# NVlabs/CenterPose

Hardware: AMD Instinct MI355X
Metric: images/sec at 512x512 DLA-34 (backbone + heat-map decode + post-process + PnP) (higher is better)
Workload: dtype f32 via split-f16 (f16x3) MFMA, f32 accumulate

## Files before the change

centerpose_amd/csrc/dcn16t.hip:

```cpp
#include <type_traits>

#include "dcn_patch_common.h"
#include "patch16_common.h"
#include "upadd_common.h"

namespace {

constexpr int T_TH = PATCH_TH, T_TW = PATCH_TW, T_HALO = 3;
constexpr int T_PW = T_TW + 2 * T_HALO, T_PH = T_TH + 2 * T_HALO, T_NPIX = T_PH * T_PW;
constexpr int T_CK = 16;
constexpr int T_PSTR = T_CK * 4 + 16;
constexpr int T_ECAP = 184;
constexpr int T_NPIX_ALL = T_NPIX + T_ECAP + T_PW + 1;
constexpr int T_NSTEP = 9;
constexpr int T_RQ = T_PW * (T_CK / 4);
constexpr int T_ROUNDS = T_PH / 2;
static_assert(2 * T_RQ <= 256 && T_PH % 2 == 0, "two patch rows per staging round");
static_assert(T_NPIX_ALL * T_PSTR + T_ECAP * 24 + 64 <= 53 * 1024, "three workgroups per CU");
static_assert((T_PSTR / 16) % 2 == 1, "odd pixel pitch in bank groups");

struct TGeo {
    static constexpr int PH = T_PH, PW = T_PW, HALO = T_HALO, ECAP = T_ECAP;
    static __device__ __forceinline__ int corner(int qy, int qx) { return qy * T_PW + qx; }
    static __device__ __forceinline__ int spare(int e) { return T_NPIX + e; }
};

template <int NT, bool UPADD = false>
__global__ __launch_bounds__(256, 3) void dcn16t_kernel(const ConvParams p, const int tiles_m, const int tiles_n) {
    typedef Frag<32> F;
    typedef F::acc_t acc_t;
    static_assert(NT == 2, "64-wide N tile");
    __shared__ __attribute__((aligned(16))) unsigned char patch[T_NPIX_ALL * T_PSTR];
    __shared__ int exc_key[T_ECAP];
    __shared__ int exc_goff[T_ECAP];
    __shared__ __attribute__((aligned(16))) float exc_w[T_ECAP][4];
    __shared__ int exc_count;

    const int tid = threadIdx.x, lane = tid & 63;
    const int wid = __builtin_amdgcn_readfirstlane(tid >> 6);
    const int lrow = lane >> 5, lcol = lane & 31;
    const int tile = tile_of_block(tiles_m, tiles_n);
    const int tn = tile % tiles_n;
    int tm = tile / tiles_n;
    const int txs = p.W / T_TW, tys = p.H / T_TH;
    const int tx0 = (tm % txs) * T_TW;
    tm /= txs;
    const int ty0 = (tm % tys) * T_TH, b = tm / tys;
    const AmaxRaw amax_raw = conv_in_scale_issue(p);
    const unsigned img_px = (unsigned)p.B * p.H * p.W;
    const __amdgpu_buffer_rsrc_t r_x = make_rsrc(p.src[0], img_px * (unsigned)p.Cin * 4u);
    const __amdgpu_buffer_rsrc_t r_om = make_rsrc(p.offmask, img_px * 128u);
    const unsigned w_bytes = (unsigned)((size_t)p.CoutPad * p.Kpad16 * 2);
    const __amdgpu_buffer_rsrc_t r_wh = make_rsrc(p.w16f_hi, w_bytes), r_wl = make_rsrc(p.w16f_lo, w_bytes);
    const int cb = p.Cin * 4, rowb = p.W * cb;
    auto stage_geo = [&](int t, int* goff, int* lds, int* row0, bool* col_ok) {
        const int rp = t >= T_RQ ? 1 : 0, within = t - rp * T_RQ, col = within >> 2;
        const int gx = tx0 - T_HALO + col;
        *row0 = ty0 - T_HALO + rp;
        *col_ok = t < 2 * T_RQ && (unsigned)gx < (unsigned)p.W;
        *goff = ((b * p.H + *row0) * p.W + gx) * cb + (within & 3) * 16;
        *lds = (rp * T_PW + col) * T_PSTR + (within & 3) * 16;
    };
    auto stage_issue = [&](float4 (&sv)[T_ROUNDS], int goff, int row0, bool col_ok, int csoff) {
#pragma unroll
        for (int k = 0; k < T_ROUNDS; ++k) {
            const bool ok = col_ok && (unsigned)(row0 + 2 * k) < (unsigned)p.H;
            sv[k] = buf_ld4s(r_x, ok ? (unsigned)(goff + 2 * k * rowb) : OOB, csoff);
        }
    };
    auto stage_store = [&](const float4 (&sv)[T_ROUNDS], int lds, int t) {
        if (t < 2 * T_RQ) {
#pragma unroll
            for (int k = 0; k < T_ROUNDS; ++k) *reinterpret_cast<float4*>(patch + lds + k * (2 * T_PW * T_PSTR)) = sv[k];
        }
    };

    if (tid == 0) exc_count = 0;
    for (int i = tid; i < (T_NPIX_ALL - T_NPIX) * (T_PSTR / 16); i += 256)
        *reinterpret_cast<float4*>(patch + T_NPIX * T_PSTR + i * 16) = make_float4(0.f, 0.f, 0.f, 0.f);
    const int y = ty0 + 2 * wid + patch_perm_row(lcol), x = tx0 + patch_perm_col(lcol);
    const unsigned rec = (unsigned)((b * p.H + y) * p.W + x) * 128u;
    float od[12], omk[5];
    dcn_load_record(r_om, rec, lrow, od, omk);
    float4 sv0[T_ROUNDS];
    int g0_off, g0_lds, g0_row;
    bool g0_ok;
    stage_geo(tid, &g0_off, &g0_lds, &g0_row, &g0_ok);
    stage_issue(sv0, g0_off, g0_row, g0_ok, 0);
    float afwd, ainv;
    conv_in_scale_finish(p, amax_raw, &afwd, &ainv);
    afwd = __uint_as_float(__builtin_amdgcn_readfirstlane(__float_as_uint(afwd)));
    ainv = __uint_as_float(__builtin_amdgcn_readfirstlane(__float_as_uint(ainv)));
    __syncthreads();

    uint32_t sq[5], sw[5][4];
    const DcnExcList exc = {exc_key, exc_goff, &exc_w[0][0], &exc_count};
    dcn_setup_taps<TGeo>(od, omk, lrow, y, x, ty0, tx0, b, p.H, p.W, cb, afwd, exc, sq, sw);
    int addr[9];
    f32x2 bw[9][2];
    dcn_expand_taps<T_PSTR>(sq, sw, lrow, addr, bw);
    stage_store(sv0, g0_lds, tid);
    __syncthreads();
    const int nexc_all = __builtin_amdgcn_readfirstlane(exc_count);
    const bool slow = nexc_all > T_ECAP;
    const int nexc = nexc_all < T_ECAP ? nexc_all : T_ECAP;

    const int G = p.Kpad16 / 16, gpt = p.Cin / 16;
    const int nch = p.Cin / T_CK;
    unsigned b_voff[NT];
#pragma unroll
    for (int j = 0; j < NT; ++j) b_voff[j] = (unsigned)(((tn * NT + j) * G) * 1024 + lane * 16);
    u32x4 wbh[2][NT], wbl[2][NT];
    auto issue_w = [&](int set, int ch, int u) {
        int so = (u * gpt + ch) * 1024;
        if (u >= T_NSTEP) so = ch + 1 < nch ? ((u - T_NSTEP) * gpt + ch + 1) * 1024 : 0x7ffffff0;
#pragma unroll
        for (int j = 0; j < NT; ++j) {
            wbh[set][j] = __builtin_amdgcn_raw_buffer_load_b128(r_wh, (int)b_voff[j], so, 0);
            wbl[set][j] = __builtin_amdgcn_raw_buffer_load_b128(r_wl, (int)b_voff[j], so, 0);
        }
    };

    acc_t acc[1][NT];
#pragma unroll
    for (int j = 0; j < NT; ++j)
#pragma unroll
        for (int r = 0; r < F::NACC; ++r) acc[0][j][r] = 0.f;

    auto mma_step = [&](const float4 (&r)[4][2], const f32x2 (&w)[2], const u32x4 (&bh)[NT], const u32x4 (&bl)[NT], auto&& mid) {
        h8 ah, al;
        dcn_blend_split(r, w, &ah, &al);
        __builtin_amdgcn_sched_barrier(0);
        mid();
        __builtin_amdgcn_sched_barrier(0);
        dcn_mma3<true, NT>(acc[0], ah, al, bh, bl);
    };

    if (!slow) {
        auto gather = [&](float4 (&r)[4][2], int a) {
            const unsigned char* ap = patch + a;
#pragma unroll
            for (int c = 0; c < 4; ++c) {
                const int co = ((c >> 1) * T_PW + (c & 1)) * T_PSTR;
                r[c][0] = *reinterpret_cast<const float4*>(ap + co);
                r[c][1] = *reinterpret_cast<const float4*>(ap + co + 16);
            }
        };
        auto stage_exceptions = [&](int csoff, int t) {
            dcn_stage_exceptions<T_CK / 4, T_PSTR>(t, nexc, exc, r_x, p.H, p.W, cb, rowb, csoff, patch + T_NPIX * T_PSTR);
        };
        auto chunk = [&](auto par_c, int ch) {
            constexpr int PAR = decltype(par_c)::value;
            const int csoff = ch * (T_CK * 4);
            const int t = lane_opaque(tid);
            if (ch > 0) {
                __syncthreads();
                float4 sv[T_ROUNDS];
                int goff, lds, row0;
                bool col_ok;
                stage_geo(t, &goff, &lds, &row0, &col_ok);
                stage_issue(sv, goff, row0, col_ok, csoff);
                stage_exceptions(csoff, t);
                stage_store(sv, lds, t);
            } else {
                stage_exceptions(csoff, t);
            }
            __syncthreads();
            float4 raw[4][2];
            gather(raw, addr[0]);
#pragma unroll
            for (int u = 0; u < T_NSTEP; ++u) {
                issue_w((PAR + u + 1) & 1, ch, u + 1);
                __builtin_amdgcn_sched_barrier(0);
                mma_step(raw, bw[u], wbh[(PAR + u) & 1], wbl[(PAR + u) & 1], [&]() {
                    if (u + 1 < T_NSTEP) gather(raw, addr[u + 1]);
                });
                __builtin_amdgcn_sched_barrier(0);
            }
        };
        issue_w(0, 0, 0);
        for (int ch = 0; ch < nch; ch += 2) {
            chunk(std::integral_constant<int, 0>(), ch);
            chunk(std::integral_constant<int, 1>(), ch + 1);
        }
    } else {
        dcn_setup_global(r_om, rec, y, x, b, p.H, p.W, cb, afwd, addr, bw);
        for (int ch = 0; ch < nch; ++ch) {
#pragma unroll
            for (int u = 0; u < T_NSTEP; ++u) {
                float4 r[4][2];
                const int so = ch * (T_CK * 4);
                issue_w(0, ch, u);
                dcn_gather_global(r_x, addr[u], lrow, rowb, cb, so, r);
                __builtin_amdgcn_sched_barrier(0);
                mma_step(r, bw[u], wbh[0], wbl[0], []() {});
                __builtin_amdgcn_sched_barrier(0);
            }
        }
    }
    {
        const int ln = lane_opaque((int)__builtin_amdgcn_mbcnt_hi(~0u, __builtin_amdgcn_mbcnt_lo(~0u, 0u))), h4 = ln >> 5, lc = ln & 31;
        const int pix0 = __builtin_amdgcn_readfirstlane((b * p.H + ty0 + 2 * wid) * p.W + tx0);
        const __amdgpu_buffer_rsrc_t ro = make_rsrc(p.out + (size_t)pix0 * p.ldo + p.coff, (unsigned)((p.W + T_TW) * p.ldo) * 4u);
        const __amdgpu_buffer_rsrc_t r_sc = make_rsrc(p.scale, (unsigned)p.CoutPad * 4u), r_sh = make_rsrc(p.shift, (unsigned)p.CoutPad * 4u);
        const unsigned vpix = (unsigned)((patch_perm_row(lc) * p.W + patch_perm_col(lc)) * p.ldo) * 4u;
        const int nb0 = tn * (32 * NT);
        const bool relu = p.act == CP_ACT_RELU;
        float amax = 0.f;
        constexpr int U_WSTR = 64 * 4 + 32;
        __amdgpu_buffer_rsrc_t r_t = r_sc;
        unsigned u_toff[2][2];
        int u_woff[2][2];
        if constexpr (UPADD) {
            const int f = p.up_f, k = 2 * f, Ht = p.H / f, Wt = p.W / f, ntap = k * k;
            static_assert(T_NPIX_ALL * T_PSTR >= 64 * U_WSTR, "the f = 4 table fits the patch");
            const int t = wid * 64 + ln;
            __syncthreads();
#pragma unroll
            for (int r = 0; r < 4; ++r) {
                const int i = t + 256 * r;
                if (i < ntap * 16)
                    *reinterpret_cast<float4*>(patch + (i >> 4) * U_WSTR + (i & 15) * 16) = reinterpret_cast<const float4*>(p.up_wt)[i];
            }
            r_t = make_rsrc(p.up_t, (unsigned)p.B * Ht * Wt * (unsigned)p.up_ld * 4u);
            int ky0, kx0, iy0, ix0;
            cp_upadd_axis(ty0 + 2 * wid + patch_perm_row(lc), f, &ky0, &iy0);
            cp_upadd_axis(tx0 + patch_perm_col(lc), f, &kx0, &ix0);
#pragma unroll
            for (int a = 0; a < 2; ++a)
#pragma unroll
                for (int bb = 0; bb < 2; ++bb) {
                    const int iy = iy0 - a, ix = ix0 - bb;
                    const bool ok = (unsigned)iy < (unsigned)Ht && (unsigned)ix < (unsigned)Wt;
                    u_toff[a][bb] = ok ? (unsigned)(((b * Ht + iy) * Wt + ix) * p.up_ld) * 4u + 16u * h4 : OOB_BASE;
                    u_woff[a][bb] = ((ky0 + a * f) * k + kx0 + bb * f) * U_WSTR + 16 * h4;
                }
            __syncthreads();
        }
#pragma unroll
        for (int j = 0; j < NT; ++j)
#pragma unroll
            for (int g4 = 0; g4 < 4; ++g4) {
                const int nsc = (nb0 + 32 * j + 8 * g4) * 4;
                const float4 sc = p.scale ? buf_ld4s(r_sc, (unsigned)(16 * h4), nsc) : make_float4(1.f, 1.f, 1.f, 1.f);
                const float4 sh = p.shift ? buf_ld4s(r_sh, (unsigned)(16 * h4), nsc) : make_float4(0.f, 0.f, 0.f, 0.f);
                float v[4] = {acc[0][j][4 * g4] * (sc.x * ainv) + sh.x, acc[0][j][4 * g4 + 1] * (sc.y * ainv) + sh.y,
                              acc[0][j][4 * g4 + 2] * (sc.z * ainv) + sh.z, acc[0][j][4 * g4 + 3] * (sc.w * ainv) + sh.w};
                if (relu) {
#pragma unroll
                    for (int i = 0; i < 4; ++i) v[i] = fmaxf(v[i], 0.f);
                }
                if constexpr (UPADD) {
                    float4 tv[2][2], wv[2][2];
#pragma unroll
                    for (int a = 0; a < 2; ++a)
#pragma unroll
                        for (int bb = 0; bb < 2; ++bb) {
                            tv[a][bb] = buf_ld4s(r_t, u_toff[a][bb], nsc);
                            wv[a][bb] = *reinterpret_cast<const float4*>(patch + u_woff[a][bb] + (32 * j + 8 * g4) * 4);
                        }
                    const float4 u = cp_upadd_piece(tv, wv, make_float4(v[0], v[1], v[2], v[3]));
                    v[0] = u.x; v[1] = u.y; v[2] = u.z; v[3] = u.w;
                }
                const int n0 = nb0 + 32 * j + 8 * g4 + 4 * h4;
                const bool n_ok = n0 < p.Cout;
#pragma unroll
                for (int i = 0; i < 4; ++i) amax = fmaxf(amax, n_ok ? fabsf(v[i]) : 0.f);
                const u32x4 pk4 = {__float_as_uint(v[0]), __float_as_uint(v[1]), __float_as_uint(v[2]), __float_as_uint(v[3])};
                __builtin_amdgcn_raw_buffer_store_b128(pk4, ro, (int)(n_ok ? vpix + (unsigned)n0 * 4u : 0x80000000u), 0, 0);
            }
        if (p.out_amax) cp_amax_commit(p.out_amax, amax);
    }
}

}

bool cp_dcn16t_supported(const ConvParams& p) { return cp_dcn16s_supported(p); }

bool cp_dcn16t_upadd_supported(const ConvParams& p) {
    return cp_dcn16t_supported(p) && p.up_t && p.up_wt && (p.up_f == 2 || p.up_f == 4) && p.Cout == 64 && p.CoutPad == 64 &&
           p.ldo == 64 && p.coff == 0 && p.up_ld >= 64 && p.up_ld % 4 == 0 && p.H % p.up_f == 0 && p.W % p.up_f == 0 &&
           (size_t)p.B * (p.H / p.up_f) * (p.W / p.up_f) * p.up_ld * 4 < (size_t)0xf0000000u;
}

int cp_launch_dcn16t(const ConvParams& p, hipStream_t stream) {
    if (!cp_dcn16t_supported(p) || (p.up_t && !cp_dcn16t_upadd_supported(p))) return CP_ERR_INVALID;
    const int tiles_m = p.B * (p.H / T_TH) * (p.W / T_TW), tiles_n = p.CoutPad / 64;
    if (p.up_t) hipLaunchKernelGGL((dcn16t_kernel<2, true>), dim3(tiles_m * tiles_n), dim3(256), 0, stream, p, tiles_m, tiles_n);
    else hipLaunchKernelGGL((dcn16t_kernel<2>), dim3(tiles_m * tiles_n), dim3(256), 0, stream, p, tiles_m, tiles_n);
    return hipGetLastError() == hipSuccess ? CP_OK : CP_ERR_LAUNCH;
}
```

centerpose_amd/csrc/patch16_common.h:

```cpp
#pragma once
#include "igemm16_common.h"

namespace {

constexpr int PATCH_TH = 8, PATCH_TW = 16;

__device__ __forceinline__ int patch_perm_row(int m) { return (0x96 >> (m >> 2)) & 1; }
__device__ __forceinline__ int patch_perm_col(int m) { return 4 * (m >> 3) + (m & 3); }

template <int MT, int NT, int WM, int WN, bool PERM = false>
__device__ __forceinline__ void patch_epilogue(const ConvParams& p, Frag<32>::acc_t (&acc)[MT][NT], int b, int ty0, int tx0,
                                               int tn, int wm, int wn, int lane, float ainv) {
    typedef Frag<32> F;
    constexpr int TW = PATCH_TW;
    constexpr int BN = 32 * NT * WN;
    const int lcol = lane & 31;
    const int act = p.act;
    const bool has_res = p.res != nullptr, has_gn = p.gn_stats != nullptr;
    float amax = 0.f;
    const int h4 = lane >> 5;
#pragma unroll
    for (int j = 0; j < NT; ++j) {
        const int n = tn * BN + wn * (NT * 32) + j * 32 + lcol;
        const float sc = (p.scale ? p.scale[n] : 1.f) * ainv;
        const float sh = p.shift ? p.shift[n] : 0.f;
        const bool n_ok = n < p.Cout;
        const bool sig_lane = act == CP_ACT_SIGMOID || (act == CP_ACT_SIGMOID_FROM && n >= p.act_from);
#pragma unroll
        for (int i = 0; i < MT; ++i) {
            const int m0 = wm * (MT * 32) + i * 32;
            const int pix0 = __builtin_amdgcn_readfirstlane((b * p.H + ty0 + (m0 >> 4)) * p.W + tx0);
            float v[F::NACC];
#pragma unroll
            for (int r = 0; r < F::NACC; ++r) v[r] = acc[i][j][r] * sc + sh;
            if (has_res) {
                const __amdgpu_buffer_rsrc_t rr = make_rsrc(p.res + (size_t)pix0 * p.res_ld, (unsigned)((p.W + TW) * p.res_ld) * 4u);
                const unsigned vr = n_ok ? (unsigned)((PERM ? h4 * p.W : 4 * h4) * p.res_ld + n) * 4u : 0x80000000u;
                const unsigned vr1 = n_ok ? (unsigned)((1 - h4) * p.W * p.res_ld + n) * 4u : 0x80000000u;
#pragma unroll
                for (int r = 0; r < F::NACC; ++r) {
                    const int so = PERM ? (4 * (r >> 2) + (r & 3)) * p.res_ld * 4
                                        : (((r >> 3) * p.W) + 8 * ((r >> 2) & 1) + (r & 3)) * p.res_ld * 4;
                    const bool flip = PERM && ((0x6 >> (r >> 2)) & 1);
                    v[r] += __uint_as_float(__builtin_amdgcn_raw_buffer_load_b32(rr, (int)(flip ? vr1 : vr), so, 0));
                }
            }
            if (act == CP_ACT_RELU) {
#pragma unroll
                for (int r = 0; r < F::NACC; ++r) v[r] = fmaxf(v[r], 0.f);
            } else if (act == CP_ACT_SIGMOID || act == CP_ACT_SIGMOID_FROM) {
#pragma unroll
                for (int r = 0; r < F::NACC; ++r) v[r] = sig_lane ? 1.f / (1.f + expf(-v[r])) : v[r];
            }
#pragma unroll
            for (int r = 0; r < F::NACC; ++r) amax = fmaxf(amax, fabsf(v[r]));
            if (has_gn) {
                float s1 = 0.f, s2 = 0.f;
                if (n_ok) {
#pragma unroll
                    for (int r = 0; r < F::NACC; ++r) { s1 += v[r]; s2 += v[r] * v[r]; }
                }
#pragma unroll
                for (int o = 1; o < 8; o <<= 1) { s1 += __shfl_xor(s1, o, 64); s2 += __shfl_xor(s2, o, 64); }
                s1 += __shfl_xor(s1, 32, 64);
                s2 += __shfl_xor(s2, 32, 64);
                if ((lane & 7) == 0 && lane < 32 && n_ok) {
                    double* st = p.gn_stats + ((size_t)b * p.gn_groups + n / p.gn_cpg) * 2;
                    atomicAdd(st, (double)s1);
                    atomicAdd(st + 1, (double)s2);
                }
            }
            float* frag_out = p.out + (size_t)pix0 * p.ldo + p.coff;
            const __amdgpu_buffer_rsrc_t ro = make_rsrc(frag_out, (unsigned)((p.W + TW) * p.ldo) * 4u);
            const unsigned vo = n_ok ? (unsigned)((PERM ? h4 * p.W : 4 * h4) * p.ldo + n) * 4u : 0x80000000u;
            const unsigned vo1 = n_ok ? (unsigned)((1 - h4) * p.W * p.ldo + n) * 4u : 0x80000000u;
#pragma unroll
            for (int r = 0; r < F::NACC; ++r) {
                const int so = PERM ? (4 * (r >> 2) + (r & 3)) * p.ldo * 4
                                    : (((r >> 3) * p.W) + 8 * ((r >> 2) & 1) + (r & 3)) * p.ldo * 4;
                const bool flip = PERM && ((0x6 >> (r >> 2)) & 1);
                __builtin_amdgcn_raw_buffer_store_b32(__float_as_uint(v[r]), ro, (int)(flip ? vo1 : vo), so, 0);
            }
        }
    }
    if (p.out_amax) cp_amax_commit(p.out_amax, amax);
}

}
```

Before: 4538.

## Batch epilogue loads ahead of compute in DCN and patch16 conv epilogues

The DCN epilogue now issues all scale/shift loads, the upsample weight-table loads and the up-tensor loads in batches before consuming them. For f=2 the weight table is staged into a dedicated LDS region during the prologue, overlapping with the first weight fetch, which removes two barriers from the epilogue. The patch16 epilogue hoists the residual loads for all fragments ahead of the math and defers stores until after they are consumed. This trades higher register pressure and extra LDS (16 rows of table) for exposing more memory-level parallelism, and could hurt occupancy.

```diff
diff --git a/centerpose_amd/csrc/dcn16t.hip b/centerpose_amd/csrc/dcn16t.hip
--- a/centerpose_amd/csrc/dcn16t.hip
+++ b/centerpose_amd/csrc/dcn16t.hip
@@ -13,10 +13,11 @@
 constexpr int T_ECAP = 184;
 constexpr int T_NPIX_ALL = T_NPIX + T_ECAP + T_PW + 1;
 constexpr int T_NSTEP = 9;
+constexpr int U_WSTR = 64 * 4 + 32;
 constexpr int T_RQ = T_PW * (T_CK / 4);
 constexpr int T_ROUNDS = T_PH / 2;
 static_assert(2 * T_RQ <= 256 && T_PH % 2 == 0, "two patch rows per staging round");
-static_assert(T_NPIX_ALL * T_PSTR + T_ECAP * 24 + 64 <= 53 * 1024, "three workgroups per CU");
+static_assert(T_NPIX_ALL * T_PSTR + T_ECAP * 24 + 64 + 16 * U_WSTR <= 53 * 1024, "three workgroups per CU");
 static_assert((T_PSTR / 16) % 2 == 1, "odd pixel pitch in bank groups");
 
 struct TGeo {
@@ -30,12 +31,13 @@
     typedef Frag<32> F;
     typedef F::acc_t acc_t;
     static_assert(NT == 2, "64-wide N tile");
-    __shared__ __attribute__((aligned(16))) unsigned char patch[T_NPIX_ALL * T_PSTR];
+    __shared__ __attribute__((aligned(16))) unsigned char patch[T_NPIX_ALL * T_PSTR + (UPADD ? 16 * U_WSTR : 0)];
     __shared__ int exc_key[T_ECAP];
     __shared__ int exc_goff[T_ECAP];
     __shared__ __attribute__((aligned(16))) float exc_w[T_ECAP][4];
     __shared__ int exc_count;
 
+    unsigned char* const up_tab = patch + T_NPIX_ALL * T_PSTR;
     const int tid = threadIdx.x, lane = tid & 63;
     const int wid = __builtin_amdgcn_readfirstlane(tid >> 6);
     const int lrow = lane >> 5, lcol = lane & 31;
@@ -136,6 +138,16 @@
         dcn_mma3<true, NT>(acc[0], ah, al, bh, bl);
     };
 
+    auto tab_fill = [&](auto&& between) {
+        if constexpr (UPADD) {
+            const int t = lane_opaque(tid);
+            const float4 q = buf_ld4(make_rsrc(p.up_wt, p.up_f == 2 ? 16u * 64u * 4u : 0u), (unsigned)t * 16u);
+            between();
+            *reinterpret_cast<float4*>(up_tab + (t >> 4) * U_WSTR + (t & 15) * 16) = q;
+        } else {
+            between();
+        }
+    };
     if (!slow) {
         auto gather = [&](float4 (&r)[4][2], int a) {
             const unsigned char* ap = patch + a;
@@ -178,13 +190,15 @@
                 __builtin_amdgcn_sched_barrier(0);
             }
         };
-        issue_w(0, 0, 0);
+        tab_fill([&]() { issue_w(0, 0, 0); });
         for (int ch = 0; ch < nch; ch += 2) {
             chunk(std::integral_constant<int, 0>(), ch);
             chunk(std::integral_constant<int, 1>(), ch + 1);
         }
     } else {
         dcn_setup_global(r_om, rec, y, x, b, p.H, p.W, cb, afwd, addr, bw);
+        tab_fill([]() {});
+        if constexpr (UPADD) __syncthreads();
         for (int ch = 0; ch < nch; ++ch) {
 #pragma unroll
             for (int u = 0; u < T_NSTEP; ++u) {
@@ -202,30 +216,24 @@
         const int ln = lane_opaque((int)__builtin_amdgcn_mbcnt_hi(~0u, __builtin_amdgcn_mbcnt_lo(~0u, 0u))), h4 = ln >> 5, lc = ln & 31;
         const int pix0 = __builtin_amdgcn_readfirstlane((b * p.H + ty0 + 2 * wid) * p.W + tx0);
         const __amdgpu_buffer_rsrc_t ro = make_rsrc(p.out + (size_t)pix0 * p.ldo + p.coff, (unsigned)((p.W + T_TW) * p.ldo) * 4u);
-        const __amdgpu_buffer_rsrc_t r_sc = make_rsrc(p.scale, (unsigned)p.CoutPad * 4u), r_sh = make_rsrc(p.shift, (unsigned)p.CoutPad * 4u);
+        const bool has_sc = p.scale != nullptr;
+        const __amdgpu_buffer_rsrc_t r_sc = make_rsrc(p.scale, has_sc ? (unsigned)p.CoutPad * 4u : 0u),
+                                     r_sh = make_rsrc(p.shift, p.shift ? (unsigned)p.CoutPad * 4u : 0u);
         const unsigned vpix = (unsigned)((patch_perm_row(lc) * p.W + patch_perm_col(lc)) * p.ldo) * 4u;
         const int nb0 = tn * (32 * NT);
         const bool relu = p.act == CP_ACT_RELU;
         float amax = 0.f;
-        constexpr int U_WSTR = 64 * 4 + 32;
         __amdgpu_buffer_rsrc_t r_t = r_sc;
         unsigned u_toff[2][2];
         int u_woff[2][2];
         if constexpr (UPADD) {
-            const int f = p.up_f, k = 2 * f, Ht = p.H / f, Wt = p.W / f, ntap = k * k;
+            const int f = p.up_f, k = 2 * f, Ht = p.H / f, Wt = p.W / f;
             static_assert(T_NPIX_ALL * T_PSTR >= 64 * U_WSTR, "the f = 4 table fits the patch");
-            const int t = wid * 64 + ln;
-            __syncthreads();
-#pragma unroll
-            for (int r = 0; r < 4; ++r) {
-                const int i = t + 256 * r;
-                if (i < ntap * 16)
-                    *reinterpret_cast<float4*>(patch + (i >> 4) * U_WSTR + (i & 15) * 16) = reinterpret_cast<const float4*>(p.up_wt)[i];
-            }
             r_t = make_rsrc(p.up_t, (unsigned)p.B * Ht * Wt * (unsigned)p.up_ld * 4u);
             int ky0, kx0, iy0, ix0;
             cp_upadd_axis(ty0 + 2 * wid + patch_perm_row(lc), f, &ky0, &iy0);
             cp_upadd_axis(tx0 + patch_perm_col(lc), f, &kx0, &ix0);
+            const int tab0 = f == 2 ? T_NPIX_ALL * T_PSTR : 0;
 #pragma unroll
             for (int a = 0; a < 2; ++a)
 #pragma unroll
@@ -233,40 +241,99 @@
                     const int iy = iy0 - a, ix = ix0 - bb;
                     const bool ok = (unsigned)iy < (unsigned)Ht && (unsigned)ix < (unsigned)Wt;
                     u_toff[a][bb] = ok ? (unsigned)(((b * Ht + iy) * Wt + ix) * p.up_ld) * 4u + 16u * h4 : OOB_BASE;
-                    u_woff[a][bb] = ((ky0 + a * f) * k + kx0 + bb * f) * U_WSTR + 16 * h4;
+                    u_woff[a][bb] = tab0 + ((ky0 + a * f) * k + kx0 + bb * f) * U_WSTR + 16 * h4;
                 }
-            __syncthreads();
+        }
+        float4 scq[NT][4], shq[NT][4];
+        auto issue_scsh = [&](int j) {
+#pragma unroll
+            for (int g4 = 0; g4 < 4; ++g4) {
+                scq[j][g4] = buf_ld4s(r_sc, (unsigned)(16 * h4), (nb0 + 32 * j + 8 * g4) * 4);
+                shq[j][g4] = buf_ld4s(r_sh, (unsigned)(16 * h4), (nb0 + 32 * j + 8 * g4) * 4);
+            }
+        };
+        auto finish = [&](int j, int g4) {
+            const float4 sh = shq[j][g4];
+            const float4 sc = has_sc ? scq[j][g4] : make_float4(1.f, 1.f, 1.f, 1.f);
+            float v[4] = {acc[0][j][4 * g4] * (sc.x * ainv) + sh.x, acc[0][j][4 * g4 + 1] * (sc.y * ainv) + sh.y,
+                          acc[0][j][4 * g4 + 2] * (sc.z * ainv) + sh.z, acc[0][j][4 * g4 + 3] * (sc.w * ainv) + sh.w};
+            if (relu) {
+#pragma unroll
+                for (int i = 0; i < 4; ++i) v[i] = fmaxf(v[i], 0.f);
+            }
+#pragma unroll
+            for (int i = 0; i < 4; ++i) acc[0][j][4 * g4 + i] = v[i];
+        };
+        auto track = [&](int j, int g4) {
+            const bool n_ok = nb0 + 32 * j + 8 * g4 + 4 * h4 < p.Cout;
+#pragma unroll
+            for (int i = 0; i < 4; ++i) amax = fmaxf(amax, n_ok ? fabsf(acc[0][j][4 * g4 + i]) : 0.f);
+        };
+        u32x4 tab4[4];
+        const int tab_t = wid * 64 + ln;
+        if constexpr (UPADD) {
+            const __amdgpu_buffer_rsrc_t r_tab = make_rsrc(p.up_wt, p.up_f == 2 ? 0u : 64u * 64u * 4u);
+#pragma unroll
+            for (int r = 0; r < 4; ++r) tab4[r] = __builtin_amdgcn_raw_buffer_load_b128(r_tab, (tab_t + 256 * r) * 16, 0, 0);
+        }
+#pragma unroll
+        for (int j = 0; j < NT; ++j) issue_scsh(j);
+        __builtin_amdgcn_sched_barrier(0);
+        if constexpr (UPADD) {
+            if (p.up_f != 2) {
+                __syncthreads();
+#pragma unroll
+                for (int r = 0; r < 4; ++r) {
+                    const int i = tab_t + 256 * r;
+                    *reinterpret_cast<u32x4*>(patch + (i >> 4) * U_WSTR + (i & 15) * 16) = tab4[r];
+                }
+                __syncthreads();
+            }
+            __builtin_amdgcn_sched_barrier(0);
         }
 #pragma unroll
         for (int j = 0; j < NT; ++j)
 #pragma unroll
             for (int g4 = 0; g4 < 4; ++g4) {
-                const int nsc = (nb0 + 32 * j + 8 * g4) * 4;
-                const float4 sc = p.scale ? buf_ld4s(r_sc, (unsigned)(16 * h4), nsc) : make_float4(1.f, 1.f, 1.f, 1.f);
-                const float4 sh = p.shift ? buf_ld4s(r_sh, (unsigned)(16 * h4), nsc) : make_float4(0.f, 0.f, 0.f, 0.f);
-                float v[4] = {acc[0][j][4 * g4] * (sc.x * ainv) + sh.x, acc[0][j][4 * g4 + 1] * (sc.y * ainv) + sh.y,
-                              acc[0][j][4 * g4 + 2] * (sc.z * ainv) + sh.z, acc[0][j][4 * g4 + 3] * (sc.w * ainv) + sh.w};
-                if (relu) {
-#pragma unroll
-                    for (int i = 0; i < 4; ++i) v[i] = fmaxf(v[i], 0.f);
+                finish(j, g4);
+                if constexpr (!UPADD) track(j, g4);
+            }
+        if constexpr (UPADD) {
+#pragma unroll
+            for (int j = 0; j < NT; ++j) {
+                __builtin_amdgcn_sched_barrier(0);
+                float4 tv[4][2][2];
+#pragma unroll
+                for (int g4 = 0; g4 < 4; ++g4)
+#pragma unroll
+                    for (int a = 0; a < 2; ++a)
+#pragma unroll
+                        for (int bb = 0; bb < 2; ++bb) tv[g4][a][bb] = buf_ld4s(r_t, u_toff[a][bb], (nb0 + 32 * j + 8 * g4) * 4);
+                __builtin_amdgcn_sched_barrier(0);
+#pragma unroll
+                for (int g4 = 0; g4 < 4; ++g4) {
+                    float4 wv[2][2];
+#pragma unroll
+                    for (int a = 0; a < 2; ++a)
+#pragma unroll
+                        for (int bb = 0; bb < 2; ++bb)
+                            wv[a][bb] = *reinterpret_cast<const float4*>(patch + u_woff[a][bb] + (32 * j + 8 * g4) * 4);
+                    const float4 u = cp_upadd_piece(tv[g4], wv, make_float4(acc[0][j][4 * g4], acc[0][j][4 * g4 + 1],
+                                                                            acc[0][j][4 * g4 + 2], acc[0][j][4 * g4 + 3]));
+                    acc[0][j][4 * g4] = u.x; acc[0][j][4 * g4 + 1] = u.y; acc[0][j][4 * g4 + 2] = u.z; acc[0][j][4 * g4 + 3] = u.w;
+                    track(j, g4);
                 }
-                if constexpr (UPADD) {
-                    float4 tv[2][2], wv[2][2];
-#pragma unroll
-                    for (int a = 0; a < 2; ++a)
-#pragma unroll
-                        for (int bb = 0; bb < 2; ++bb) {
-                            tv[a][bb] = buf_ld4s(r_t, u_toff[a][bb], nsc);
-                            wv[a][bb] = *reinterpret_cast<const float4*>(patch + u_woff[a][bb] + (32 * j + 8 * g4) * 4);
-                        }
-                    const float4 u = cp_upadd_piece(tv, wv, make_float4(v[0], v[1], v[2], v[3]));
-                    v[0] = u.x; v[1] = u.y; v[2] = u.z; v[3] = u.w;
-                }
+            }
+        }
+        __builtin_amdgcn_sched_barrier(0);
+#pragma unroll
+        for (int j = 0; j < NT; ++j)
+#pragma unroll
+            for (int g4 = 0; g4 < 4; ++g4) {
                 const int n0 = nb0 + 32 * j + 8 * g4 + 4 * h4;
                 const bool n_ok = n0 < p.Cout;
-#pragma unroll
-                for (int i = 0; i < 4; ++i) amax = fmaxf(amax, n_ok ? fabsf(v[i]) : 0.f);
-                const u32x4 pk4 = {__float_as_uint(v[0]), __float_as_uint(v[1]), __float_as_uint(v[2]), __float_as_uint(v[3])};
+                const u32x4 pk4 = {__float_as_uint(acc[0][j][4 * g4]), __float_as_uint(acc[0][j][4 * g4 + 1]),
+                                   __float_as_uint(acc[0][j][4 * g4 + 2]), __float_as_uint(acc[0][j][4 * g4 + 3])};
                 __builtin_amdgcn_raw_buffer_store_b128(pk4, ro, (int)(n_ok ? vpix + (unsigned)n0 * 4u : 0x80000000u), 0, 0);
             }
         if (p.out_amax) cp_amax_commit(p.out_amax, amax);
diff --git a/centerpose_amd/csrc/patch16_common.h b/centerpose_amd/csrc/patch16_common.h
--- a/centerpose_amd/csrc/patch16_common.h
+++ b/centerpose_amd/csrc/patch16_common.h
@@ -19,31 +19,70 @@
     const bool has_res = p.res != nullptr, has_gn = p.gn_stats != nullptr;
     float amax = 0.f;
     const int h4 = lane >> 5;
+    auto chan = [&](int j) { return tn * BN + wn * (NT * 32) + j * 32 + lcol; };
+    auto frag_pix0 = [&](int i) {
+        const int m0 = wm * (MT * 32) + i * 32;
+        return __builtin_amdgcn_readfirstlane((b * p.H + ty0 + (m0 >> 4)) * p.W + tx0);
+    };
+    float scv[NT], shv[NT];
 #pragma unroll
     for (int j = 0; j < NT; ++j) {
-        const int n = tn * BN + wn * (NT * 32) + j * 32 + lcol;
-        const float sc = (p.scale ? p.scale[n] : 1.f) * ainv;
-        const float sh = p.shift ? p.shift[n] : 0.f;
-        const bool n_ok = n < p.Cout;
-        const bool sig_lane = act == CP_ACT_SIGMOID || (act == CP_ACT_SIGMOID_FROM && n >= p.act_from);
+        scv[j] = p.scale ? p.scale[chan(j)] : 1.f;
+        shv[j] = p.shift ? p.shift[chan(j)] : 0.f;
+    }
+    float rv[MT][NT][F::NACC];
+    if (has_res) {
 #pragma unroll
-        for (int i = 0; i < MT; ++i) {
-            const int m0 = wm * (MT * 32) + i * 32;
-            const int pix0 = __builtin_amdgcn_readfirstlane((b * p.H + ty0 + (m0 >> 4)) * p.W + tx0);
-            float v[F::NACC];
+        for (int j = 0; j < NT; ++j) {
+            const int n = chan(j);
+            const bool n_ok = n < p.Cout;
+            const unsigned vr = n_ok ? (unsigned)((PERM ? h4 * p.W : 4 * h4) * p.res_ld + n) * 4u : 0x80000000u;
+            const unsigned vr1 = n_ok ? (unsigned)((1 - h4) * p.W * p.res_ld + n) * 4u : 0x80000000u;
 #pragma unroll
-            for (int r = 0; r < F::NACC; ++r) v[r] = acc[i][j][r] * sc + sh;
-            if (has_res) {
-                const __amdgpu_buffer_rsrc_t rr = make_rsrc(p.res + (size_t)pix0 * p.res_ld, (unsigned)((p.W + TW) * p.res_ld) * 4u);
-                const unsigned vr = n_ok ? (unsigned)((PERM ? h4 * p.W : 4 * h4) * p.res_ld + n) * 4u : 0x80000000u;
-                const unsigned vr1 = n_ok ? (unsigned)((1 - h4) * p.W * p.res_ld + n) * 4u : 0x80000000u;
+            for (int i = 0; i < MT; ++i) {
+                const __amdgpu_buffer_rsrc_t rr =
+                    make_rsrc(p.res + (size_t)frag_pix0(i) * p.res_ld, (unsigned)((p.W + TW) * p.res_ld) * 4u);
 #pragma unroll
                 for (int r = 0; r < F::NACC; ++r) {
                     const int so = PERM ? (4 * (r >> 2) + (r & 3)) * p.res_ld * 4
                                         : (((r >> 3) * p.W) + 8 * ((r >> 2) & 1) + (r & 3)) * p.res_ld * 4;
                     const bool flip = PERM && ((0x6 >> (r >> 2)) & 1);
-                    v[r] += __uint_as_float(__builtin_amdgcn_raw_buffer_load_b32(rr, (int)(flip ? vr1 : vr), so, 0));
+                    rv[i][j][r] = __uint_as_float(__builtin_amdgcn_raw_buffer_load_b32(rr, (int)(flip ? vr1 : vr), so, 0));
                 }
+            }
+        }
+    }
+    __builtin_amdgcn_sched_barrier(0);
+    auto store_frag = [&](int i, int j) {
+        const int n = chan(j);
+        const bool n_ok = n < p.Cout;
+        float* frag_out = p.out + (size_t)frag_pix0(i) * p.ldo + p.coff;
+        const __amdgpu_buffer_rsrc_t ro = make_rsrc(frag_out, (unsigned)((p.W + TW) * p.ldo) * 4u);
+        const unsigned vo = n_ok ? (unsigned)((PERM ? h4 * p.W : 4 * h4) * p.ldo + n) * 4u : 0x80000000u;
+        const unsigned vo1 = n_ok ? (unsigned)((1 - h4) * p.W * p.ldo + n) * 4u : 0x80000000u;
+#pragma unroll
+        for (int r = 0; r < F::NACC; ++r) {
+            const int so = PERM ? (4 * (r >> 2) + (r & 3)) * p.ldo * 4
+                                : (((r >> 3) * p.W) + 8 * ((r >> 2) & 1) + (r & 3)) * p.ldo * 4;
+            const bool flip = PERM && ((0x6 >> (r >> 2)) & 1);
+            __builtin_amdgcn_raw_buffer_store_b32(__float_as_uint(acc[i][j][r]), ro, (int)(flip ? vo1 : vo), so, 0);
+        }
+    };
+#pragma unroll
+    for (int j = 0; j < NT; ++j) {
+        const int n = chan(j);
+        const float sc = scv[j] * ainv;
+        const float sh = shv[j];
+        const bool n_ok = n < p.Cout;
+        const bool sig_lane = act == CP_ACT_SIGMOID || (act == CP_ACT_SIGMOID_FROM && n >= p.act_from);
+#pragma unroll
+        for (int i = 0; i < MT; ++i) {
+            F::acc_t& v = acc[i][j];
+#pragma unroll
+            for (int r = 0; r < F::NACC; ++r) v[r] = v[r] * sc + sh;
+            if (has_res) {
+#pragma unroll
+                for (int r = 0; r < F::NACC; ++r) v[r] += rv[i][j][r];
             }
             if (act == CP_ACT_RELU) {
 #pragma unroll
@@ -70,18 +109,15 @@
                     atomicAdd(st + 1, (double)s2);
                 }
             }
-            float* frag_out = p.out + (size_t)pix0 * p.ldo + p.coff;
-            const __amdgpu_buffer_rsrc_t ro = make_rsrc(frag_out, (unsigned)((p.W + TW) * p.ldo) * 4u);
-            const unsigned vo = n_ok ? (unsigned)((PERM ? h4 * p.W : 4 * h4) * p.ldo + n) * 4u : 0x80000000u;
-            const unsigned vo1 = n_ok ? (unsigned)((1 - h4) * p.W * p.ldo + n) * 4u : 0x80000000u;
+            if (!has_res) store_frag(i, j);
+        }
+    }
+    if (has_res) {
+        __builtin_amdgcn_sched_barrier(0);
 #pragma unroll
-            for (int r = 0; r < F::NACC; ++r) {
-                const int so = PERM ? (4 * (r >> 2) + (r & 3)) * p.ldo * 4
-                                    : (((r >> 3) * p.W) + 8 * ((r >> 2) & 1) + (r & 3)) * p.ldo * 4;
-                const bool flip = PERM && ((0x6 >> (r >> 2)) & 1);
-                __builtin_amdgcn_raw_buffer_store_b32(__float_as_uint(v[r]), ro, (int)(flip ? vo1 : vo), so, 0);
-            }
-        }
+        for (int j = 0; j < NT; ++j)
+#pragma unroll
+            for (int i = 0; i < MT; ++i) store_frag(i, j);
     }
     if (p.out_amax) cp_amax_commit(p.out_amax, amax);
 }
```

Result: no change. 4517 (-0.5%).
